# QhelDIV/ShapeFormer

Measured on AMD Instinct MI355X. Metric: shapes/sec completed (64^3 VQDIF + 512-tok AR sample + 128^3 SDF extract), higher is better.
Workload: dtype f32; 1 GPU; shape completion, 384 shapes/GPU/step: VQDIF-16 encode of 16384-pt partial cloud -> tokens -> CondTupleGPT 20+4 layers d1024 prefill + 512 KV-cached decode steps (top_k 100, top_p 0.4, early exit off) -> UNet3D+Upsampler -> 128^3 SDF query; batch_per_gpu=384, micro_batches=4, ar_steps=512, decode_res=128, parallelism=shard1, weights=hash-generated (no checkpoints ship)

## Files before the change

include/sfmi.h:

```cpp
#ifndef SFMI_H
#define SFMI_H
#include <stddef.h>
#ifdef __cplusplus
extern "C" {
#endif

#define SFMI_OK 0
#define SFMI_EINVAL (-1)
#define SFMI_ELDS (-4)
#define SFMI_ENOBLAS (-3)

int sfmi_version(void);
int sfmi_stream_spin(long long ticks, void* stream);
int sfmi_stream_create_cumask(const unsigned* mask, int words, void** stream_out);
int sfmi_stream_destroy(void* stream);
int sfmi_hwid_probe(unsigned* out, int blocks, int threads, long long ticks, void* stream);
int sfmi_tune_set(const char* name, int value);
int sfmi_tune_get(const char* name);
int sfmi_tune_generation(void);

size_t sfmi_enc_pack_floats(void);
int sfmi_enc_pack_weights(const float* fc_pos_w, const float* fc_pos_b, const float* fc0_w, const float* fc0_b,
                          const float* fc1_w, const float* fc1_b, const float* sc_w, const float* fc_c_w,
                          const float* fc_c_b, float* out);
// ... 77 lines not shown
int sfmi_decode_gemm_f32(const float* x, const float* Wp16, const float* c1, const float* c2, const float* resid, float* out,
                         int M, int N, int K, int ldo, int ln, int act, int out_packed, int S, float* slab, int* cnt, void* stream);
int sfmi_decode_gemm_prof_f32(const float* x, const float* Wp16, const float* c1, const float* c2, const float* resid, float* out,
                              int M, int N, int K, int ldo, int ln, int act, int out_packed, int S, float* slab, int* cnt, int* pblk,
                              unsigned long long* prof, void* stream);
int sfmi_decode_gemm_live_f32(const float* x, const float* Wp16, const float* c1, const float* c2, const float* resid, float* out,
                              int M, int N, int K, int ldo, int ln, int act, int out_packed, int S, float* slab, int* cnt,
                              const int* alen, void* stream);
int sfmi_gpt_compact_rows_f32(const int* alen, int* slot_of, int* row_of, int* nlive, int* slot_len, const float* stage, float* resid,
                              int B, int Bpad, int D, void* stream);
int sfmi_decode_gemm_rows_f32(const float* x, const float* Wp16, const float* c1, const float* c2, const float* resid, float* out,
                              int M, int N, int K, int ldo, int ln, int act, int out_packed, int S, float* slab, int* cnt,
                              const int* nlive, int partial, void* stream);
int sfmi_gpt_embed_rows_f32(const float* E0, const float* E1, const float* Ex, const float* pos_emb, const float* cond_pos_emb,
                            const int* seq, const int* len, const int* Lc, float* stage, int B, int D, int Lmax, int end0, void* stream);
int sfmi_gpt_embed_packed_f32(const float* E0, const float* E1, const float* Ex, const float* pos_emb, const float* cond_pos_emb,
                              const int* seq, const int* len, const int* Lc, float* resid, int B, int D, int Lmax, int end0,
                              void* stream);
int sfmi_gpt_attn_decode_f32(const float* qkv_packed, const float* unused, float* Kc, float* Vc, const int* len, float* y_packed,
                             int S, int B, int D, int H, int Lmax, const int* shared_len, void* stream);
int sfmi_gpt_attn_decode_gated_f32(const float* qkv_packed, float* Kc, float* Vc, const int* len, float* y_packed, int B, int D, int H,
                                   int Lmax, const int* shared_len, int* sem, int* blk, int lanes, unsigned long long* prof,
                                   void* stream);
int sfmi_gpt_attn_decode_rows_f32(const float* qkv_packed, float* Kc, float* Vc, const int* slot_len, const int* row_of, float* y_packed,
                                  int B, int D, int H, int Lmax, const int* shared_len, int* sem, int* blk, int lanes,
                                  unsigned long long* prof, void* stream);
int sfmi_gpt_sample_f32(const float* part, int* seq, int* len, const int* Lc, float* logp, float* hist, const int* force,
                        float* resid, const float* E0, const float* E1, const float* Ex, const float* pos_emb, int D, int S,
                        int B, int V, int ldv, int Lmax, int tuple_i, int end0, int end1, int top_k, float top_p,
                        float temperature, int greedy_row0, int mask_invalid, int mask_completion, int max_steps,
// ... 199 lines not shown
```

shapeformer_amd/_lib.py:

```python
from __future__ import annotations

import ctypes as C
import os

_HERE = os.path.dirname(os.path.abspath(__file__))
LIB_PATH = os.path.join(_HERE, "lib", "libsfmi.so")

_lib = None
SFMI_OK, SFMI_EINVAL = 0, -1

c_f32p = C.c_void_p
c_ptr = C.c_void_p
i32, i64, sz, f32 = C.c_int, C.c_longlong, C.c_size_t, C.c_float

PROTOTYPES = {
    "sfmi_version": (i32, []),
    "sfmi_stream_spin": (i32, [i64, c_ptr]),
    "sfmi_stream_create_cumask": (i32, [c_ptr, i32, c_ptr]),
    "sfmi_stream_destroy": (i32, [c_ptr]),
    "sfmi_hwid_probe": (i32, [c_ptr, i32, i32, i64, c_ptr]),
    "sfmi_tune_set": (i32, [C.c_char_p, i32]),
    "sfmi_tune_get": (i32, [C.c_char_p]),
    "sfmi_tune_generation": (i32, []),
    "sfmi_relu_bwd_f32": (i32, [c_ptr, c_ptr, c_ptr, i64, c_ptr]),
# ... 74 lines not shown
                                c_ptr]),
    "sfmi_sgemm_mfma_f32": (i32, [i32] * 5 + [c_ptr, i32, c_ptr, i32, c_ptr, i32, i32, c_ptr, i32, c_ptr, c_ptr, i64, f32, C.c_uint, c_ptr]),
    "sfmi_ce_rows_f32": (i32, [c_ptr, c_ptr, c_ptr, i64, i32, i32, c_ptr]),
    "sfmi_gpt_attn_decode_f32": (i32, [c_ptr] * 6 + [i32] * 5 + [c_ptr, c_ptr]),
    "sfmi_gpt_attn_decode_gated_f32": (i32, [c_ptr] * 5 + [i32] * 4 + [c_ptr, c_ptr, c_ptr, i32, c_ptr, c_ptr]),
    "sfmi_gpt_attn_prefill_f32": (i32, [c_ptr] * 5 + [i32] * 5 + [c_ptr, f32, C.c_uint, c_ptr]),
    "sfmi_gpt_attn_prefill_lse_f32": (i32, [c_ptr] * 5 + [i32] * 5 + [c_ptr, f32, C.c_uint, c_ptr, c_ptr]),
    "sfmi_gpt_sample_f32": (i32, [c_ptr] * 12 + [i32] * 10 + [C.c_float, C.c_float] + [i32] * 4 + [C.c_uint, c_ptr, i32, i32, i32, i32, c_ptr]),
    "sfmi_gpt_sample_live_f32": (i32, [c_ptr] * 12 + [i32] * 10 + [C.c_float, C.c_float] + [i32] * 4 + [C.c_uint, c_ptr, i32, i32, i32, i32, c_ptr, i32,
                                       c_ptr]),
    "sfmi_gpt_mask_logits_f32": (i32, [c_ptr] * 5 + [i32] * 9 + [c_ptr]),
    "sfmi_decode_gemm_f32": (i32, [c_ptr] * 6 + [i32] * 8 + [c_ptr, c_ptr, c_ptr]),
    "sfmi_decode_gemm_live_f32": (i32, [c_ptr] * 6 + [i32] * 8 + [c_ptr, c_ptr, c_ptr, c_ptr]),
    "sfmi_decode_gemm_rows_f32": (i32, [c_ptr] * 6 + [i32] * 8 + [c_ptr, c_ptr, c_ptr, i32, c_ptr]),
    "sfmi_gpt_compact_rows_f32": (i32, [c_ptr] * 7 + [i32] * 3 + [c_ptr]),
    "sfmi_gpt_embed_rows_f32": (i32, [c_ptr] * 9 + [i32] * 4 + [c_ptr]),
    "sfmi_gpt_attn_decode_rows_f32": (i32, [c_ptr] * 6 + [i32] * 4 + [c_ptr, c_ptr, c_ptr, i32, c_ptr, c_ptr]),
    "sfmi_gpt_sample_rows_f32": (i32, [c_ptr] * 11 + [i32] * 10 + [C.c_float, C.c_float] + [i32] * 3 + [C.c_uint, c_ptr, i32, i32, i32, i32, c_ptr, c_ptr,
                                       c_ptr]),
    "sfmi_decode_gemm_prof_f32": (i32, [c_ptr] * 6 + [i32] * 8 + [c_ptr, c_ptr, c_ptr, c_ptr, c_ptr]),
    "sfmi_decode_gemm_slab_floats": (sz, [i32, i32, i32]),
    "sfmi_gpt_embed_packed_f32": (i32, [c_ptr] * 9 + [i32] * 4 + [c_ptr]),
    "sfmi_set_len_i32": (i32, [c_ptr, c_ptr, i32, i32, c_ptr]),
    "sfmi_transpose_f32": (i32, [c_ptr, c_ptr, i32, i32, i32, i32, c_ptr]),
    "sfmi_colsum_f32": (i32, [c_ptr, c_ptr, i32, i32, i32, i32, c_ptr]),
    "sfmi_colsum_slices": (i32, [i32, i32]),
    "sfmi_colsum_ws_f32": (i32, [c_ptr, c_ptr, i32, i32, i32, i32, c_ptr, c_ptr]),
    "sfmi_layernorm_bwd_scratch_floats": (sz, [i32, i32]),
    "sfmi_gelu_f32": (i32, [c_ptr, c_ptr, i64, c_ptr]),
    "sfmi_gelu_bwd_f32": (i32, [c_ptr, c_ptr, c_ptr, i64, c_ptr]),
# ... 110 lines not shown
```

shapeformer_amd/csrc/gpt.hip:

```cpp
#include "sfmi_common.h"
#include <mutex>
#include <type_traits>
#include <string>

#define MFMA(a, b, c) __builtin_amdgcn_mfma_f32_32x32x2f32((a), (b), (c), 0, 0, 0)

#define g_tune g_sfmi_tune


struct RowPrepArgs {
  const float *E0, *E1, *Ex, *pos_emb, *cond_pos_emb;
  const int *seq, *len, *Lc;
  const int* nval;
  const int* extra;
  int* extra_out;
  const float* resid_in;
  const float* part;
  const float* bias;
  const float* Eadd;
  float* resid_out;
  float* xn;
  const float *gamma, *beta;
  int mode, S, M, D, Lmax, P , end0;
  const int* rowoff;
// ... 992 lines not shown
  else {
    int lo = 0, hi = lc;
    while (lo < hi) { int mid = (lo + hi) >> 1; if (row[2 * mid] > pos) hi = mid; else lo = mid + 1; }
    ext = row[2 * (lo < lc ? lo : lc - 1)];
  }
  const f32x4* e0 = reinterpret_cast<const f32x4*>(E0 + (long long)pos * D);
  const f32x4* e1 = reinterpret_cast<const f32x4*>(E1 + (long long)val * D);
  const f32x4* ex = reinterpret_cast<const f32x4*>(Ex + (long long)ext * D);
  const f32x4* pe = reinterpret_cast<const f32x4*>(t < lc ? cond_pos_emb + (long long)t * D : pos_emb + (long long)(t - lc) * D);
  for (int qd = tid; qd < D / 4; qd += 256)
    *reinterpret_cast<f32x4*>(row_major ? resid + (long long)b * D + 4 * qd : resid + pk_off(b, 4 * qd, D)) = ((e0[qd] + e1[qd]) + ex[qd]) + pe[qd];
}

__global__ __launch_bounds__(256) void compact_rows_kernel(const int* __restrict__ alen, int* __restrict__ slot_of, int* __restrict__ row_of,
                                                           int* __restrict__ nlive, int* __restrict__ slot_len,
                                                           const float* __restrict__ stage, float* __restrict__ resid, int B, int Bpad, int D) {
  __shared__ int s_all[4], s_below[4], s_mine;
  const int b = blockIdx.x, tid = threadIdx.x, lane = tid & 63, wave = tid >> 6;
  const int al = tid < B ? alen[tid] : -1;
  const unsigned long long m_all = __ballot(al >= 0), m_below = __ballot(al >= 0 && tid < b);
  if (lane == 0) { s_all[wave] = __popcll(m_all); s_below[wave] = __popcll(m_below); }
  if (tid == b) s_mine = al;
  __syncthreads();
  const int total = (s_all[0] + s_all[1]) + (s_all[2] + s_all[3]), below = (s_below[0] + s_below[1]) + (s_below[2] + s_below[3]);
  const int mine = s_mine;
  const int slot = mine >= 0 ? below : total + (b - below);
  if (tid == 0) {
    slot_of[b] = mine >= 0 ? slot : -1;
    row_of[slot] = b;
    slot_len[slot] = mine >= 0 ? mine : -1;
    if (b == 0) *nlive = total;
  }
  if (b == 0 && B + tid < Bpad) { row_of[B + tid] = -1; slot_len[B + tid] = -1; }
  for (int qd = tid; qd < D / 4; qd += 256) {
    f32x4 v = {0.f, 0.f, 0.f, 0.f};
    if (mine >= 0) v = *reinterpret_cast<const f32x4*>(stage + (long long)b * D + 4 * qd);
    *reinterpret_cast<f32x4*>(resid + pk_off(slot, 4 * qd, D)) = v;
  }
}

__global__ __launch_bounds__(256) void ce_rows_kernel(const float* __restrict__ logits, const int* __restrict__ target,
                                                      float* __restrict__ loss, int V, int ld) {
  __shared__ float red[8];
  const int m = blockIdx.x, tid = threadIdx.x, lane = tid & 63, wave = tid >> 6;
  const float* row = logits + (long long)m * ld;
  float mx = -INFINITY;
// ... 35 lines not shown
  __syncthreads();
  if (part == 0) {
    double a = 0.0, b = 0.0;
    for (int q = 0; q < 16; ++q) { a += p1[r][q]; b += p2[r][q]; }
    if (n < N && bias) b += (double)bias[n];
    c1[nt * 16 + r] = (float)a;
    c2[nt * 16 + r] = (float)b;
  }
}

__global__ void set_len_kernel(int* len, const int* src, int B, int delta) {
  int i = blockIdx.x * blockDim.x + threadIdx.x;
  if (i < B) len[i] = src[i] + delta;
}

template <class P>
static int decode_gemm_launch(const float* x, const float* Wp16, const float* c1, const float* c2, const float* resid, float* out, int M,
                              int N, int K, int ldo, int ln, int act, int out_packed, int S, float* slab, int* cnt, int* pblk,
                              unsigned long long* prof, void* stream, const int* alen = nullptr, const int* nlive = nullptr, int partial = 0) {
  if (prof && (alen || nlive)) return SFMI_EINVAL;
  if (!x || !Wp16 || !out || M <= 0 || M > 192 || S <= 0 || K % S || (ln && !c1)) return SFMI_EINVAL;
  if (out_packed && N % 16) return SFMI_EINVAL;
  if (!out_packed && (ldo < N || ldo % 4)) return SFMI_EINVAL;
  if (S > 1 && (!slab || !cnt)) return SFMI_EINVAL;
  if (prof && !pblk) return SFMI_EINVAL;
  const int kslice = K / S;
  const int tiles = (M + 15) / 16;
  int groups = (tiles + 5) / 6, MT = (tiles + groups - 1) / groups;
  int NWv = (kslice >= 2048 && MT <= 4) ? 16 : 8;
  const int knob_nw = g_tune.dgemm_nw;
  if ((knob_nw == 4 || knob_nw == 8 || knob_nw == 16) && kslice % (16 * knob_nw) == 0 && MT <= (knob_nw == 8 ? 6 : 4)) NWv = knob_nw;
  if (kslice % (16 * NWv)) NWv = kslice % 64 == 0 ? 4 : 1;
  if (kslice % (16 * NWv)) return SFMI_EINVAL;
  const int mt_cap = NWv == 1 ? 1 : NWv == 4 ? 4 : 6;
  if (MT > mt_cap) { groups = (tiles + mt_cap - 1) / mt_cap; MT = (tiles + groups - 1) / groups; }
  DGemmArgs a;
  a.x = x; a.Wp = Wp16; a.c1 = c1; a.c2 = c2; a.resid = resid; a.out = out; a.M = M; a.N = N; a.K = K; a.ldo = ldo; a.ln = ln; a.act = act;
  a.out_packed = out_packed; a.slab = slab; a.cnt = cnt; a.pblk = pblk; a.prof = prof; a.prio = g_tune.dgemm_prio; a.alen = alen;
  a.nlive = nlive; a.partial = partial;
  hipStream_t st = (hipStream_t)stream;
  if ((g_tune.dgemm_nt2 == 2 || (g_tune.dgemm_nt2 == 1 && tiles % 3 == 0)) && NWv == 8 && (kslice / 8 / 16) % 2 == 0 && tiles >= 3) {
    const int g2 = (tiles + 2) / 3, MT2 = (tiles + g2 - 1) / g2;
    dim3 grid2(((N + 15) / 16 + 1) / 2, S, g2);
#define DG2(MT_) hipLaunchKernelGGL((dgemm_kernel<MT_, 8, 2, 2, P>), grid2, dim3(512), 0, st, a)
    if (MT2 == 2) DG2(2); else DG2(3);
#undef DG2
    SFMI_CHECK_LAUNCH();
    return SFMI_OK;
  }
  dim3 grid((N + 15) / 16, S, groups);
  const int steps = kslice / NWv / 16;
  int un = MT == 1 ? 8 : (MT == 2 ? 4 : (MT <= 5 ? 2 : 1));
  if (g_tune.dgemm_un > 0 && g_tune.dgemm_un < un) un = g_tune.dgemm_un;
  while (un & (un - 1)) un &= un - 1;
  while (un > 1 && steps % un) un >>= 1;
#define DG(MT_, NW_, UN_) hipLaunchKernelGGL((dgemm_kernel<MT_, NW_, UN_, 1, P>), grid, dim3(64 * NW_), 0, st, a)
#define DGU8(MT_, NW_) do { if (un >= 8) DG(MT_, NW_, 8); else if (un >= 4) DG(MT_, NW_, 4); else if (un >= 2) DG(MT_, NW_, 2); else DG(MT_, NW_, 1); } while (0)
#define DGU4(MT_, NW_) do { if (un >= 4) DG(MT_, NW_, 4); else if (un >= 2) DG(MT_, NW_, 2); else DG(MT_, NW_, 1); } while (0)
#define DGU2(MT_, NW_) do { if (un >= 2) DG(MT_, NW_, 2); else DG(MT_, NW_, 1); } while (0)
  if (NWv == 16) { if (MT == 1) DGU8(1, 16); else if (MT == 2) DGU4(2, 16); else if (MT == 3) DGU2(3, 16); else DGU2(4, 16); }
  else if (NWv == 4) {
    if (MT == 1) DG(1, 4, 1); else if (MT == 2) DG(2, 4, 1);
    else if (MT == 3) DGU2(3, 4);
    else DGU2(4, 4);
// ... 67 lines not shown
int sfmi_gpt_embed_f32(const float* E0, const float* E1, const float* Ex, const float* pos_emb, const float* cond_pos_emb,
                       const int* seq, const int* len, const int* Lc, const int* nval, const int* extra, int* extra_out,
                       float* resid_out, float* xn, const float* gamma, const float* beta, int B, int P, int D, int Lmax,
                       int end0, const int* rowoff, int M_packed, void* stream) {
  if (!E0 || !E1 || !Ex || !pos_emb || !cond_pos_emb || !seq || !len || !Lc || D % 4 || D > 4096) return SFMI_EINVAL;
  if (rowoff && (P <= 0 || M_packed <= 0)) return SFMI_EINVAL;
  RowPrepArgs a = {};
  a.E0 = E0; a.E1 = E1; a.Ex = Ex; a.pos_emb = pos_emb; a.cond_pos_emb = cond_pos_emb; a.seq = seq; a.len = len; a.Lc = Lc;
  a.nval = nval; a.extra = extra; a.extra_out = extra_out;
  a.resid_out = resid_out; a.xn = xn; a.gamma = gamma; a.beta = beta; a.mode = 0; a.M = P ? B * P : B; a.D = D; a.Lmax = Lmax;
  a.P = P; a.end0 = end0; a.rowoff = rowoff; a.nB = B;
  if (rowoff) a.M = M_packed;
  hipLaunchKernelGGL(rowprep_kernel, dim3(a.M), dim3(256), 0, (hipStream_t)stream, a);
  SFMI_CHECK_LAUNCH();
  return SFMI_OK;
}

int sfmi_gpt_rowprep_f32(const float* resid_in, const float* part, const float* bias, const float* Eadd, const int* seq,
                         const int* len, const int* Lc, const int* nval, float* resid_out, float* xn, const float* gamma,
                         const float* beta, int S, int M, int P, int D, int Lmax, const int* rowoff, int B, void* stream) {
  if (!resid_in || D % 4 || D > 4096 || (Eadd && (!seq || !len)) || (rowoff && B <= 0)) return SFMI_EINVAL;
  RowPrepArgs a = {};
  a.resid_in = resid_in; a.part = part; a.bias = bias; a.Eadd = Eadd; a.seq = seq; a.len = len; a.Lc = Lc; a.nval = nval;
  a.resid_out = resid_out; a.xn = xn; a.gamma = gamma; a.beta = beta; a.mode = 1; a.S = S; a.M = M; a.D = D; a.Lmax = Lmax; a.P = P;
  a.rowoff = rowoff; a.nB = B;
  hipLaunchKernelGGL(rowprep_kernel, dim3(M), dim3(256), 0, (hipStream_t)stream, a);
  SFMI_CHECK_LAUNCH();
  return SFMI_OK;
}

// ... 151 lines not shown
  return SFMI_OK;
}
int sfmi_gpt_embed_rows_f32(const float* E0, const float* E1, const float* Ex, const float* pos_emb, const float* cond_pos_emb,
                            const int* seq, const int* len, const int* Lc, float* stage, int B, int D, int Lmax, int end0, void* stream) {
  if (!E0 || !E1 || !Ex || !pos_emb || !cond_pos_emb || !seq || !len || !Lc || !stage || D % 16) return SFMI_EINVAL;
  hipLaunchKernelGGL(embed_packed_kernel, dim3(B), dim3(256), 0, (hipStream_t)stream, E0, E1, Ex, pos_emb, cond_pos_emb, seq, len, Lc,
                     stage, D, Lmax, end0, 1);
  SFMI_CHECK_LAUNCH();
  return SFMI_OK;
}
int sfmi_gpt_compact_rows_f32(const int* alen, int* slot_of, int* row_of, int* nlive, int* slot_len, const float* stage, float* resid,
                              int B, int Bpad, int D, void* stream) {
  if (!alen || !slot_of || !row_of || !nlive || !slot_len || !stage || !resid || B <= 0 || B > 256 || Bpad < B || Bpad - B > 256 || D % 16)
    return SFMI_EINVAL;
  hipLaunchKernelGGL(compact_rows_kernel, dim3(B), dim3(256), 0, (hipStream_t)stream, alen, slot_of, row_of, nlive, slot_len, stage, resid,
                     B, Bpad, D);
  SFMI_CHECK_LAUNCH();
  return SFMI_OK;
}

int sfmi_ce_rows_f32(const float* logits, const int* target, float* loss, long long M, int V, int ld, void* stream) {
  if (!logits || !target || !loss || M <= 0 || V <= 0) return SFMI_EINVAL;
  hipLaunchKernelGGL(ce_rows_kernel, dim3((unsigned)M), dim3(256), 0, (hipStream_t)stream, logits, target, loss, V, ld);
  SFMI_CHECK_LAUNCH();
  return SFMI_OK;
}

int sfmi_set_len_i32(int* len, const int* src, int B, int delta, void* stream) {
  if (!len || !src) return SFMI_EINVAL;
  hipLaunchKernelGGL(set_len_kernel, dim3((B + 63) / 64), dim3(64), 0, (hipStream_t)stream, len, src, B, delta);
  SFMI_CHECK_LAUNCH();
// ... 5 lines not shown
```

shapeformer_amd/gpt.py:

```python
from __future__ import annotations

import os
import numpy as np
import torch

from . import _lib as L
from . import weights as W


def _t(sd, k, dev):
    v = sd[k]
    if isinstance(v, np.ndarray):
        v = torch.from_numpy(v)
    return v.to(dev, torch.float32).contiguous()


def pack_skinny16(w: torch.Tensor) -> torch.Tensor:
    N, K = w.shape
    NT = (N + 15) // 16
    if NT * 16 != N:
        w = torch.cat([w, w.new_zeros(NT * 16 - N, K)], 0)
    return w.view(NT, 16, K // 16, 4, 4).permute(0, 2, 3, 1, 4).contiguous().view(-1)


class _Layer:
    pass


class CondTupleGPT:
    S_PROJ, S_FC2 = 1, 4
    S_PROJ_M = 1
    PREFILL_ON_CHAIN_STREAMS = True
    PREFILL_BLAS_ROWS = 2048 if os.environ.get("SFMI_ROCBLAS") == "1" else None
    PREFILL_TILE_KERNEL = False

    def _blas(self):
        if not hasattr(self, "_has_blas"):
            self._has_blas = bool(L.lib().sfmi_blas_available())
        return self._has_blas

    def __init__(self, state_dict=None, n_embd=1024, n_head=16, n_layers=(20, 4), block_size=812,
# ... 112 lines not shown

    def mark_decode_weights_stale(self):
        self._decode_stale = True

    def _alloc(self, B, max_steps, slot=0):
        key = (B, max_steps)
        if not hasattr(self, "_states"):
            self._states, self._graphs = {}, {}
        cur = self._states.get(slot)
        if cur is not None and cur["key"] == key:
            self._state = cur
            return cur
        dev, D = self.dev, self.D
        f = lambda *shape: torch.empty(shape, device=dev, dtype=torch.float32)
        Bp = int(L.lib().sfmi_decode_gemm_padded_rows(B))
        st = dict(key=key,
                  seq=torch.zeros(B, self.Lmax + 1, 2, device=dev, dtype=torch.int32),
                  len=torch.zeros(B, device=dev, dtype=torch.int32), Lc=torch.zeros(B, device=dev, dtype=torch.int32),
                  alen=torch.zeros(B, device=dev, dtype=torch.int32),
                  resid=torch.zeros(Bp, D, device=dev), qkv=torch.zeros(Bp, 3 * D, device=dev), y=torch.zeros(Bp, D, device=dev),
                  h=torch.zeros(Bp, 4 * D, device=dev), logit=f(B, self.Vpad),
                  emb=torch.zeros(B, D, device=dev), slot_of=torch.zeros(B, device=dev, dtype=torch.int32),
                  row_of=torch.zeros(Bp, device=dev, dtype=torch.int32), slot_len=torch.zeros(Bp, device=dev, dtype=torch.int32),
                  nlive=torch.zeros(1, device=dev, dtype=torch.int32),
                  slab=f(L.lib().sfmi_decode_gemm_slab_floats(Bp, 4 * D, 4)), cnt=torch.zeros(Bp // 16 * (max(4 * D, self.Vpad) // 16 + 1), device=dev, dtype=torch.int32),
                  Kc=f(len(self.layers), B, self.Lmax + 1, D), Vc=f(len(self.layers), B, self.Lmax + 1, D),
                  logp=torch.zeros(B, max_steps, 2, device=dev, dtype=torch.float32),
                  blk=torch.zeros(1, device=dev, dtype=torch.int32),
                  pblk=torch.zeros(1, device=dev, dtype=torch.int32),
                  prof=self._prof_zero(dev),
                  shared=torch.zeros(1, device=dev, dtype=torch.int32),
                  seed=torch.zeros(1, device=dev, dtype=torch.int32))
        self._state = st
        self._states[slot] = st
        self._graphs.pop(slot, None)
        return st

    @staticmethod
    def _prof_zero(dev):
# ... 3 lines not shown
        return t

    def launch_profile(self, reset=True):
        out = {}
        sts = [st for st in self._states.values() if "prof" in st]
        for i, fam in enumerate(("attn", "gemm")):
            n = sum(int(st["prof"][4 * i + 2].item()) for st in sts)
            tk = sum(int(st["prof"][4 * i + 1].item()) for st in sts)
            out[fam] = (n, tk * 0.01 / n if n else 0.0)
        if reset:
            for st in sts:
                st["prof"].copy_(self._prof_zero(self.dev))
                st["pblk"].zero_()
        return out

    def _dgemm(self, x, wp, c1, c2, resid, out, M, N, K, ldo, ln, act, packed=1, S=1, st=None, prof=False, alen=None, nlive=None, partial=1):
        st = st or self._state
        while S > 1 and (K // S) % 128:
            S //= 2
        slab, cnt = (L.ptr(st["slab"]), L.ptr(st["cnt"])) if S > 1 else (None, None)
        if nlive is not None and not prof:
            L.check(L.lib().sfmi_decode_gemm_rows_f32(L.ptr(x), L.ptr(wp), L.ptr(c1), L.ptr(c2), L.ptr(resid), L.ptr(out), M, N, K, ldo,
                                                      ln, act, packed, S, slab, cnt, L.ptr(nlive), int(partial), L.stream_ptr()), "sfmi_decode_gemm_rows_f32")
            return
        if alen is not None and not prof:
            L.check(L.lib().sfmi_decode_gemm_live_f32(L.ptr(x), L.ptr(wp), L.ptr(c1), L.ptr(c2), L.ptr(resid), L.ptr(out), M, N, K, ldo,
                                                      ln, act, packed, S, slab, cnt, L.ptr(alen), L.stream_ptr()), "sfmi_decode_gemm_live_f32")
            return
        if prof:
            L.check(L.lib().sfmi_decode_gemm_prof_f32(L.ptr(x), L.ptr(wp), L.ptr(c1), L.ptr(c2), L.ptr(resid), L.ptr(out), M, N, K, ldo,
                                                      ln, act, packed, S, slab, cnt, L.ptr(st["pblk"]), L.ptr(st["prof"][4:]),
                                                      L.stream_ptr()), "sfmi_decode_gemm_prof_f32")
            return
        L.check(L.lib().sfmi_decode_gemm_f32(L.ptr(x), L.ptr(wp), L.ptr(c1), L.ptr(c2), L.ptr(resid), L.ptr(out), M, N, K, ldo,
                                             ln, act, packed, S, slab, cnt, L.stream_ptr()), "sfmi_decode_gemm_f32")
# ... 150 lines not shown
            M = lg.shape[0] * lg.shape[1]
            tgt = z[..., i].contiguous().view(-1)
            rows = torch.empty(M, device=self.dev, dtype=torch.float32)
            L.check(L.lib().sfmi_ce_rows_f32(L.ptr(lg), L.ptr(tgt), L.ptr(rows), M, self.V, self.V, L.stream_ptr()), "sfmi_ce_rows_f32")
            loss = loss + rows.mean()
        return loss / 2

    ATTN_LANES = 2
    MAX_CHAIN_ROWS = 192
    SHARED_PREFIX_MIN_ROW_TOKENS = 2800
    SINGLE_CHAIN_ROWS = 96
    SKIP_ENDED = True
    SKIP_ENDED_GEMM = True
    COMPACT_LIVE = True
    COMPACT_LIVE_TILES = True

    def decode_step(self, st, B, sp):
        D = self.D
        lib = L.lib()
        r = st["resid"]
        skip = self._ablate
        if "@" in skip:
            skip = ",".join(t.split("@")[0] for t in skip.split(",") if int(t.split("@")[1]) == sp.get("chain", 0))
        lanes = int(sp.get("gate_lanes", 0))
        pa, pg = "attn" in self._profile, "gemm" in self._profile
        Sqkv, Sproj, Sfc1, Sfc2, Shead = 1, self.S_PROJ if B <= 16 else self.S_PROJ_M, 1, self.S_FC2, 1
        armed = int(sp.get("skip_ended", 0))
        alen_a = st["alen"] if armed else st["len"]
        alen_g = st["alen"] if armed >= 2 else None
        compact = int(sp.get("compact_live", 0))
        gk = dict(alen=alen_g)
        if compact:
            gk = dict(nlive=st["nlive"], partial=int(compact >= 2))
            L.check(lib.sfmi_gpt_compact_rows_f32(L.ptr(st["alen"]), L.ptr(st["slot_of"]), L.ptr(st["row_of"]), L.ptr(st["nlive"]),
                                                  L.ptr(st["slot_len"]), L.ptr(st["emb"]), L.ptr(r), B, r.shape[0], D, L.stream_ptr()),
                    "sfmi_gpt_compact_rows_f32")
        for li, ly in enumerate(self.layers):
            stage_end = li + 1 == len(self.layers) or self.layers[li + 1].stage != ly.stage
            if "gemm" not in skip:
                self._dgemm(r, ly.pqkv, ly.c1qkv, ly.c2qkv, None, st["qkv"], B, 3 * D, D, 3 * D, 1, 0, S=Sqkv, st=st, prof=pg, **gk)
            if "attn" not in skip and compact:
                L.check(lib.sfmi_gpt_attn_decode_rows_f32(L.ptr(st["qkv"]), L.ptr(st["Kc"][li]), L.ptr(st["Vc"][li]),
                                                          L.ptr(st["slot_len"]), L.ptr(st["row_of"]), L.ptr(st["y"]), B, D, self.H, self.Lmax + 1,
                                                          L.ptr(st["shared"]) if sp.get("shared_prefix") else None,
                                                          L.ptr(self._sem) if lanes else None, L.ptr(st["blk"]) if (lanes or pa) else None, lanes,
                                                          L.ptr(st["prof"]) if pa else None, L.stream_ptr()), "sfmi_gpt_attn_decode_rows_f32")
            elif "attn" not in skip:
                L.check(lib.sfmi_gpt_attn_decode_gated_f32(L.ptr(st["qkv"]), L.ptr(st["Kc"][li]), L.ptr(st["Vc"][li]),
                                                           L.ptr(alen_a), L.ptr(st["y"]), B, D, self.H, self.Lmax + 1,
                                                           L.ptr(st["shared"]) if sp.get("shared_prefix") else None,
                                                           L.ptr(self._sem) if lanes else None, L.ptr(st["blk"]) if (lanes or pa) else None, lanes,
                                                           L.ptr(st["prof"]) if pa else None, L.stream_ptr()), "sfmi_gpt_attn_decode_gated_f32")
            if "gemm" not in skip:
                self._dgemm(st["y"], ly.pproj, None, ly.bproj, r, r, B, D, D, D, 0, 0, S=Sproj, st=st, prof=pg, **gk)
                self._dgemm(r, ly.pfc1, ly.c1fc1, ly.c2fc1, None, st["h"], B, 4 * D, D, 4 * D, 1, 1, S=Sfc1, st=st, prof=pg, **gk)
                self._dgemm(st["h"], ly.pfc2, None, ly.bfc2, r, r, B, D, 4 * D, D, 0, 0, S=Sfc2, st=st, prof=pg, **gk)
            if stage_end:
                s = ly.stage
# ... 24 lines not shown
    def _prepare(self, c_tokens, Lc, max_steps, sp_kw, slot=0, row_offset=0, rows_total=None, return_logits=False,
                 force_tokens=None, use_graph=True, shared_prefix=False, z_tokens=None, gate_lanes=0):
        B = c_tokens.shape[0]
        Lz = 0 if z_tokens is None else int(z_tokens.shape[1])
        if B > self.MAX_CHAIN_ROWS:
            raise L.SfmiError(f"a decode chain holds up to {self.MAX_CHAIN_ROWS} rows (larger batches run as several chains: sample / sample_microbatched)")
        self._sync_params()
        if getattr(self, "_decode_stale", False):
            self.refresh_decode_weights()
        Lc_host = Lc.cpu().tolist()
        Lc_max = max(Lc_host)
        if shared_prefix == "auto":
            shared_prefix = B * Lc_max >= self.SHARED_PREFIX_MIN_ROW_TOKENS
        steps = min(max_steps, self.Lmax - Lc_max - Lz)
        st = self._alloc(B, max_steps, slot)
        st["seq"].zero_()
        st["seq"][:, :c_tokens.shape[1]] = c_tokens.to(self.dev, torch.int32)
        st["Lc"].copy_(Lc.to(self.dev, torch.int32))
        st["len"].copy_(st["Lc"])
        if Lz:
            pos = st["Lc"].long()[:, None] + torch.arange(Lz, device=self.dev)[None, :]
            st["seq"][torch.arange(B, device=self.dev)[:, None], pos] = torch.as_tensor(z_tokens).to(self.dev, torch.int32)
            st["len"].add_(Lz)
            shared_prefix = False
        st["alen"].copy_(st["len"])
        st["slot_of"].copy_(torch.arange(B, device=self.dev, dtype=torch.int32))
        st["row_of"].fill_(-1)
        st["row_of"][:B] = st["slot_of"]
        st["slot_len"].fill_(-1)
        st["slot_len"][:B] = st["len"]
        st["nlive"].fill_(B)
        st["logp"].zero_()
        st["seed"].copy_(torch.from_numpy(np.array([sp_kw["seed"]], np.uint32).view(np.int32)))
        hist = None
        if return_logits:
            hist = [torch.full((B, max_steps, self.V), float("nan"), device=self.dev) for _ in range(2)]
        sp = dict(sp_kw, max_steps=int(max_steps), hist=hist, row_offset=int(row_offset),
                  rows_total=int(rows_total if rows_total is not None else B), chain=int(slot - 100 if slot >= 100 else 0),
                  shared_prefix=bool(shared_prefix), step_offset=Lz, gate_lanes=int(gate_lanes))
        sp["skip_ended"] = (2 if self.SKIP_ENDED_GEMM else 1) if (self.SKIP_ENDED and sp_kw["mask_invalid"] and not return_logits
                                                                  and force_tokens is None and not self._ablate) else 0
        sp["compact_live"] = (2 if self.COMPACT_LIVE_TILES else 1) if (self.COMPACT_LIVE and sp["skip_ended"] >= 2) else 0
        if force_tokens is not None:
            ft = torch.zeros(B, max_steps, 2, dtype=torch.int32)
            ft[:, :force_tokens.shape[1]] = torch.as_tensor(force_tokens).to(torch.int32)
            sp["force"] = ft.to(self.dev)
            use_graph = False
        P = Lc_max + Lz - 1
        st["nval"], st["extra"] = None, None
        if Lz:
            st["nval"] = (st["len"] - 1).contiguous()
        if shared_prefix:
            assert len(set(Lc_host)) == 1 and bool((st["seq"][:, :Lc_max] == st["seq"][:1, :Lc_max]).all()), \
                "shared_prefix needs identical condition rows"
            st["shared"].fill_(P)
            st["M_packed"] = P
            st["rowoff"] = torch.tensor([0, P], dtype=torch.int32).to(self.dev)
# ... 4 lines not shown
            nrow = [max(l + Lz - 1, 0) for l in Lc_host]
            st["M_packed"] = sum(nrow)
            st["rowoff"] = torch.tensor([0] + list(np.cumsum(nrow)), dtype=torch.int32).to(self.dev)
            if P > 0 and st["M_packed"] > 0:
                self.prefill(st, B, P)
        if sp["compact_live"]:
            L.check(L.lib().sfmi_gpt_embed_rows_f32(L.ptr(self.E[0]), L.ptr(self.E[1]), L.ptr(self.Ex), L.ptr(self.pos_emb),
                                                    L.ptr(self.cond_pos_emb), L.ptr(st["seq"]), L.ptr(st["len"]), L.ptr(st["Lc"]),
                                                    L.ptr(st["emb"]), B, self.D, self.Lmax + 1, self.end[0], L.stream_ptr()),
                    "sfmi_gpt_embed_rows_f32")
        else:
            L.check(L.lib().sfmi_gpt_embed_packed_f32(L.ptr(self.E[0]), L.ptr(self.E[1]), L.ptr(self.Ex), L.ptr(self.pos_emb),
                                                      L.ptr(self.cond_pos_emb), L.ptr(st["seq"]), L.ptr(st["len"]), L.ptr(st["Lc"]),
                                                      L.ptr(st["resid"]), B, self.D, self.Lmax + 1, self.end[0], L.stream_ptr()),
                    "sfmi_gpt_embed_packed_f32")
        graph = None
        if use_graph and steps > 1:
            gkey = (B, tuple(sorted((k, v) for k, v in sp.items() if k not in ("hist", "force", "seed"))), return_logits,
                    self._ablate, self._profile, self.S_PROJ, self.S_PROJ_M, self.S_FC2,
                    int(L.lib().sfmi_tune_generation()))
            cached = self._graphs.get(slot)
            if cached is None or cached[0] != gkey or return_logits:
                side = torch.cuda.Stream(device=self.dev)
                side.wait_stream(torch.cuda.current_stream())
                saved = {k: st[k].clone() for k in ("seq", "len", "alen", "logp", "resid", "emb")}
                with torch.cuda.stream(side):
                    self.decode_step(st, B, sp)
                torch.cuda.current_stream().wait_stream(side)
                torch.cuda.synchronize()
                for k, v in saved.items():
                    st[k].copy_(v)
                graph = torch.cuda.CUDAGraph()
                with torch.cuda.graph(graph):
                    self.decode_step(st, B, sp)
                for k, v in saved.items():
                    st[k].copy_(v)
                self._graphs[slot] = (gkey, graph)
            graph = self._graphs[slot][1]
        return dict(st=st, sp=sp, B=B, steps=steps, graph=graph, hist=hist, Lc_host=Lc_host, Lz=Lz)

    @staticmethod
    def _sp(top_k, top_p, temperature, best_in_first, mask_invalid, mask_invalid_completion, seed):
        return dict(top_k=int(top_k), top_p=float(top_p), temperature=float(temperature), best_in_first=best_in_first,
                    mask_invalid=mask_invalid, mask_invalid_completion=mask_invalid_completion,
                    seed=W._fnv1a32(f"sample-uniforms-{seed}"))

    @torch.no_grad()
    def sample(self, c_tokens, Lc, max_steps=512, top_k=100, top_p=0.4, temperature=1.0, best_in_first=True,
               mask_invalid=True, mask_invalid_completion=True, seed=0, stop_early=True, use_graph=True,
               return_logits=False, check_every=32, force_tokens=None, to_host=True, after_prefill=None, shared_prefix=False,
               z_tokens=None, row_offset=0, rows_total=None, ended_reduce=None):
        if c_tokens.shape[0] > self.SINGLE_CHAIN_ROWS:
            n_micro = min(4, -(-c_tokens.shape[0] // 80))
            r = self.sample_microbatched(c_tokens, Lc, n_micro=n_micro, max_steps=max_steps, top_k=top_k, top_p=top_p, temperature=temperature,
# ... 4 lines not shown
                                         ended_reduce=ended_reduce)
            if not to_host:
                return r
            Lz = 0 if z_tokens is None else int(z_tokens.shape[1])
            return self._host_result(r["state"], Lc.cpu().tolist(), Lz, r.get("logits_history"))
        sp_kw = self._sp(top_k, top_p, temperature, best_in_first, mask_invalid, mask_invalid_completion, seed)
        ctx = self._prepare(c_tokens, Lc, max_steps, sp_kw, return_logits=return_logits, force_tokens=force_tokens,
                            use_graph=use_graph, shared_prefix=shared_prefix, z_tokens=z_tokens, row_offset=int(row_offset),
                            rows_total=rows_total)
        ended = (lambda: self._all_ended(st, B)) if ended_reduce is None else (lambda: bool(ended_reduce(self._all_ended(st, B))))
        st, sp, B, steps, g, hist, Lc_host = (ctx[k] for k in ("st", "sp", "B", "steps", "graph", "hist", "Lc_host"))
        if after_prefill is not None:
            after_prefill()
        done = 0
        if g is not None:
            while done < steps:
                n = min(check_every, steps - done) if stop_early else steps - done
                for _ in range(n):
                    g.replay()
                done += n
                if stop_early and ended():
                    break
        else:
            while done < steps:
                self.decode_step(st, B, sp)
                done += 1
                if stop_early and (done % check_every == 0 or done == steps) and ended():
                    break
        if not to_host:
            return dict(state=st, steps=done)
        return self._host_result(st, Lc_host, ctx["Lz"], hist)

    def _host_result(self, st, Lc_host, Lz, hist):
        B = len(Lc_host)
        ln = st["len"].cpu().tolist()
# ... 124 lines not shown
        if lanes:
            for s in streams:
                cur.wait_stream(s)
            self._sem.zero_()
            for c in ctxs:
                c["st"]["blk"].zero_()
            for s in streams:
                s.wait_stream(cur)
        if after_prefill is not None:
            for s in streams:
                cur.wait_stream(s)
            after_prefill()
            for s in streams:
                s.wait_stream(cur)
        done = 0
        while done < steps:
            n = min(check_every, steps - done) if stop_early else steps - done
            for _ in range(n):
                for c, s in zip(ctxs, streams):
                    with torch.cuda.stream(s):
                        if c["graph"] is not None:
                            c["graph"].replay()
                        else:
                            self.decode_step(c["st"], c["B"], c["sp"])
            done += n
            if stop_early:
                for s in streams:
                    cur.wait_stream(s)
                e_ = all(self._all_ended(c["st"], c["B"]) for c in ctxs)
                if (e_ if ended_reduce is None else bool(ended_reduce(e_))):
                    break
        for s in streams:
            cur.wait_stream(s)
        merged = {k: torch.cat([c["st"][k] for c in ctxs], 0) for k in ("seq", "len", "Lc", "logp")}
        res = dict(state=merged, steps=done)
        if return_logits:
            res["logits_history"] = [torch.cat([c["hist"][i] for c in ctxs], 0) for i in range(2)]
        return res

    def _all_ended(self, st, B):
# ... 5 lines not shown
```

Before: 139.6 shapes/s.

## Capture per-tile-budget decode graphs and pick one from lagged live-row feedback

Captures one decode-step graph for each row-tile budget and selects the budget every 8 steps. The choice uses the live-row count read back asynchronously from two intervals earlier through a pinned ring and events. Decode GEMMs and attention then launch only the budgeted row tiles, so grid size shrinks as sequences end, instead of relying on in-kernel skipping. It adds graph capture time and memory plus periodic host event syncs. An overflow flag raises an error if live rows ever exceed the budget, which could happen if the lag assumption breaks.

```diff
diff --git a/include/sfmi.h b/include/sfmi.h
--- a/include/sfmi.h
+++ b/include/sfmi.h
@@ -115,6 +115,11 @@
                               const int* nlive, int partial, void* stream);
 int sfmi_gpt_embed_rows_f32(const float* E0, const float* E1, const float* Ex, const float* pos_emb, const float* cond_pos_emb,
                             const int* seq, const int* len, const int* Lc, float* stage, int B, int D, int Lmax, int end0, void* stream);
+int sfmi_decode_gemm_tiles_f32(const float* x, const float* Wp16, const float* c1, const float* c2, const float* resid, float* out,
+                               int form_rows, int tiles, int N, int K, int ldo, int ln, int act, int out_packed, int S, float* slab,
+                               int* cnt, const int* nlive, int partial, void* stream);
+int sfmi_gpt_compact_rows_budget_f32(const int* alen, int* slot_of, int* row_of, int* nlive, int* slot_len, const float* stage,
+                                     float* resid, int B, int Bpad, int D, int budget, int* over, void* stream);
 int sfmi_gpt_embed_packed_f32(const float* E0, const float* E1, const float* Ex, const float* pos_emb, const float* cond_pos_emb,
                               const int* seq, const int* len, const int* Lc, float* resid, int B, int D, int Lmax, int end0,
                               void* stream);
diff --git a/shapeformer_amd/_lib.py b/shapeformer_amd/_lib.py
--- a/shapeformer_amd/_lib.py
+++ b/shapeformer_amd/_lib.py
@@ -112,6 +112,8 @@
     "sfmi_decode_gemm_live_f32": (i32, [c_ptr] * 6 + [i32] * 8 + [c_ptr, c_ptr, c_ptr, c_ptr]),
     "sfmi_decode_gemm_rows_f32": (i32, [c_ptr] * 6 + [i32] * 8 + [c_ptr, c_ptr, c_ptr, i32, c_ptr]),
     "sfmi_gpt_compact_rows_f32": (i32, [c_ptr] * 7 + [i32] * 3 + [c_ptr]),
+    "sfmi_decode_gemm_tiles_f32": (i32, [c_ptr] * 6 + [i32] * 9 + [c_ptr, c_ptr, c_ptr, i32, c_ptr]),
+    "sfmi_gpt_compact_rows_budget_f32": (i32, [c_ptr] * 7 + [i32] * 4 + [c_ptr, c_ptr]),
     "sfmi_gpt_embed_rows_f32": (i32, [c_ptr] * 9 + [i32] * 4 + [c_ptr]),
     "sfmi_gpt_attn_decode_rows_f32": (i32, [c_ptr] * 6 + [i32] * 4 + [c_ptr, c_ptr, c_ptr, i32, c_ptr, c_ptr]),
     "sfmi_gpt_sample_rows_f32": (i32, [c_ptr] * 11 + [i32] * 10 + [C.c_float, C.c_float] + [i32] * 3 + [C.c_uint, c_ptr, i32, i32, i32, i32, c_ptr, c_ptr,
diff --git a/shapeformer_amd/csrc/gpt.hip b/shapeformer_amd/csrc/gpt.hip
--- a/shapeformer_amd/csrc/gpt.hip
+++ b/shapeformer_amd/csrc/gpt.hip
@@ -1030,7 +1030,8 @@
 
 __global__ __launch_bounds__(256) void compact_rows_kernel(const int* __restrict__ alen, int* __restrict__ slot_of, int* __restrict__ row_of,
                                                            int* __restrict__ nlive, int* __restrict__ slot_len,
-                                                           const float* __restrict__ stage, float* __restrict__ resid, int B, int Bpad, int D) {
+                                                           const float* __restrict__ stage, float* __restrict__ resid, int B, int Bpad, int D,
+                                                           int budget, int* __restrict__ over) {
   __shared__ int s_all[4], s_below[4], s_mine;
   const int b = blockIdx.x, tid = threadIdx.x, lane = tid & 63, wave = tid >> 6;
   const int al = tid < B ? alen[tid] : -1;
@@ -1045,7 +1046,10 @@
     slot_of[b] = mine >= 0 ? slot : -1;
     row_of[slot] = b;
     slot_len[slot] = mine >= 0 ? mine : -1;
-    if (b == 0) *nlive = total;
+    if (b == 0) {
+      *nlive = total;
+      if (over && total > 16 * budget) over[0] = 1;
+    }
   }
   if (b == 0 && B + tid < Bpad) { row_of[B + tid] = -1; slot_len[B + tid] = -1; }
   for (int qd = tid; qd < D / 4; qd += 256) {
@@ -1111,10 +1115,12 @@
   if (i < B) len[i] = src[i] + delta;
 }
 
+extern "C" int sfmi_decode_gemm_padded_rows(int M);
 template <class P>
 static int decode_gemm_launch(const float* x, const float* Wp16, const float* c1, const float* c2, const float* resid, float* out, int M,
                               int N, int K, int ldo, int ln, int act, int out_packed, int S, float* slab, int* cnt, int* pblk,
-                              unsigned long long* prof, void* stream, const int* alen = nullptr, const int* nlive = nullptr, int partial = 0) {
+                              unsigned long long* prof, void* stream, const int* alen = nullptr, const int* nlive = nullptr, int partial = 0,
+                              int budget = 0) {
   if (prof && (alen || nlive)) return SFMI_EINVAL;
   if (!x || !Wp16 || !out || M <= 0 || M > 192 || S <= 0 || K % S || (ln && !c1)) return SFMI_EINVAL;
   if (out_packed && N % 16) return SFMI_EINVAL;
@@ -1122,22 +1128,27 @@
   if (S > 1 && (!slab || !cnt)) return SFMI_EINVAL;
   if (prof && !pblk) return SFMI_EINVAL;
   const int kslice = K / S;
-  const int tiles = (M + 15) / 16;
+  int tiles = (M + 15) / 16;
   int groups = (tiles + 5) / 6, MT = (tiles + groups - 1) / groups;
   int NWv = (kslice >= 2048 && MT <= 4) ? 16 : 8;
   const int knob_nw = g_tune.dgemm_nw;
   if ((knob_nw == 4 || knob_nw == 8 || knob_nw == 16) && kslice % (16 * knob_nw) == 0 && MT <= (knob_nw == 8 ? 6 : 4)) NWv = knob_nw;
   if (kslice % (16 * NWv)) NWv = kslice % 64 == 0 ? 4 : 1;
   if (kslice % (16 * NWv)) return SFMI_EINVAL;
-  const int mt_cap = NWv == 1 ? 1 : NWv == 4 ? 4 : 6;
+  if (budget > 0) {
+    tiles = budget;
+    groups = (tiles + 5) / 6; MT = (tiles + groups - 1) / groups;
+  }
+  const int mt_cap = NWv == 1 ? 1 : (NWv == 4 || NWv == 16) ? 4 : 6;
   if (MT > mt_cap) { groups = (tiles + mt_cap - 1) / mt_cap; MT = (tiles + groups - 1) / groups; }
   DGemmArgs a;
-  a.x = x; a.Wp = Wp16; a.c1 = c1; a.c2 = c2; a.resid = resid; a.out = out; a.M = M; a.N = N; a.K = K; a.ldo = ldo; a.ln = ln; a.act = act;
+  a.x = x; a.Wp = Wp16; a.c1 = c1; a.c2 = c2; a.resid = resid; a.out = out; a.M = budget > 0 ? min(M, 16 * budget) : M; a.N = N; a.K = K; a.ldo = ldo; a.ln = ln; a.act = act;
   a.out_packed = out_packed; a.slab = slab; a.cnt = cnt; a.pblk = pblk; a.prof = prof; a.prio = g_tune.dgemm_prio; a.alen = alen;
   a.nlive = nlive; a.partial = partial;
   hipStream_t st = (hipStream_t)stream;
   if ((g_tune.dgemm_nt2 == 2 || (g_tune.dgemm_nt2 == 1 && tiles % 3 == 0)) && NWv == 8 && (kslice / 8 / 16) % 2 == 0 && tiles >= 3) {
     const int g2 = (tiles + 2) / 3, MT2 = (tiles + g2 - 1) / g2;
+    if (budget > 0 && g2 * MT2 * 16 > sfmi_decode_gemm_padded_rows(M)) return SFMI_EINVAL;
     dim3 grid2(((N + 15) / 16 + 1) / 2, S, g2);
 #define DG2(MT_) hipLaunchKernelGGL((dgemm_kernel<MT_, 8, 2, 2, P>), grid2, dim3(512), 0, st, a)
     if (MT2 == 2) DG2(2); else DG2(3);
@@ -1145,6 +1156,7 @@
     SFMI_CHECK_LAUNCH();
     return SFMI_OK;
   }
+  if (budget > 0 && groups * MT * 16 > sfmi_decode_gemm_padded_rows(M)) return SFMI_EINVAL;
   dim3 grid((N + 15) / 16, S, groups);
   const int steps = kslice / NWv / 16;
   int un = MT == 1 ? 8 : (MT == 2 ? 4 : (MT <= 5 ? 2 : 1));
@@ -1242,6 +1254,14 @@
   hipLaunchKernelGGL(rowprep_kernel, dim3(a.M), dim3(256), 0, (hipStream_t)stream, a);
   SFMI_CHECK_LAUNCH();
   return SFMI_OK;
+}
+
+int sfmi_decode_gemm_tiles_f32(const float* x, const float* Wp16, const float* c1, const float* c2, const float* resid,
+                               float* out, int form_rows, int tiles, int N, int K, int ldo, int ln, int act, int out_packed, int S,
+                               float* slab, int* cnt, const int* nlive, int partial, void* stream) {
+  if (!nlive || form_rows <= 0 || form_rows > 192 || tiles < 1 || 16 * tiles > sfmi_decode_gemm_padded_rows(form_rows)) return SFMI_EINVAL;
+  return decode_gemm_launch<DgProduct>(x, Wp16, c1, c2, resid, out, form_rows, N, K, ldo, ln, act, out_packed, S, slab, cnt, nullptr, nullptr,
+                                       stream, nullptr, nlive, partial ? 1 : 0, tiles);
 }
 
 int sfmi_gpt_rowprep_f32(const float* resid_in, const float* part, const float* bias, const float* Eadd, const int* seq,
@@ -1423,7 +1443,17 @@
   if (!alen || !slot_of || !row_of || !nlive || !slot_len || !stage || !resid || B <= 0 || B > 256 || Bpad < B || Bpad - B > 256 || D % 16)
     return SFMI_EINVAL;
   hipLaunchKernelGGL(compact_rows_kernel, dim3(B), dim3(256), 0, (hipStream_t)stream, alen, slot_of, row_of, nlive, slot_len, stage, resid,
-                     B, Bpad, D);
+                     B, Bpad, D, 0, (int*)nullptr);
+  SFMI_CHECK_LAUNCH();
+  return SFMI_OK;
+}
+int sfmi_gpt_compact_rows_budget_f32(const int* alen, int* slot_of, int* row_of, int* nlive, int* slot_len, const float* stage, float* resid,
+                                     int B, int Bpad, int D, int budget, int* over, void* stream) {
+  if (!alen || !slot_of || !row_of || !nlive || !slot_len || !stage || !resid || B <= 0 || B > 256 || Bpad < B || Bpad - B > 256 || D % 16)
+    return SFMI_EINVAL;
+  if (!over || budget < 1 || 16 * budget > Bpad) return SFMI_EINVAL;
+  hipLaunchKernelGGL(compact_rows_kernel, dim3(B), dim3(256), 0, (hipStream_t)stream, alen, slot_of, row_of, nlive, slot_len, stage, resid,
+                     B, Bpad, D, budget, over);
   SFMI_CHECK_LAUNCH();
   return SFMI_OK;
 }
diff --git a/shapeformer_amd/gpt.py b/shapeformer_amd/gpt.py
--- a/shapeformer_amd/gpt.py
+++ b/shapeformer_amd/gpt.py
@@ -25,6 +25,55 @@
 
 class _Layer:
     pass
+
+
+def tile_budget_policy(full, nlive_of_block, block, lag=2):
+    if block < lag:
+        return int(full)
+    return int(min(int(full), max(1, (int(nlive_of_block[block - lag]) + 15) // 16)))
+
+
+class _BudgetFeedback:
+    RING = 4
+
+    def __init__(self, gpt, ctxs, streams):
+        self.ctxs, self.streams, self.every = ctxs, streams, max(1, int(gpt.TILE_BUDGET_EVERY))
+        self.armed = [c.get("graphs") is not None for c in ctxs]
+        self.cur = [c["graph"] for c in ctxs]
+        self.seen = [[] for _ in ctxs]
+        if any(self.armed):
+            self.ring = [torch.zeros(self.RING, 2, dtype=torch.int32).pin_memory() if a else None for a in self.armed]
+            self.ev = [[torch.cuda.Event() for _ in range(self.RING)] if a else None for a in self.armed]
+        for c in ctxs:
+            c["budget_log"] = []
+        gpt.last_budget_log = [c["budget_log"] for c in ctxs]
+
+    def graphs(self, done):
+        if done % self.every == 0:
+            j = done // self.every
+            for i, c in enumerate(self.ctxs):
+                if not self.armed[i]:
+                    continue
+                if j >= 2:
+                    self.ev[i][(j - 2) % self.RING].synchronize()
+                    nlive, over = self.ring[i][(j - 2) % self.RING].tolist()
+                    if over:
+                        raise L.SfmiError("a decode step ran at a row-tile budget below its live rows (TILE_BUDGET)")
+                    self.seen[i].append(nlive)
+                T = tile_budget_policy((c["B"] + 15) // 16, self.seen[i], j)
+                c["budget_log"].append(T)
+                self.cur[i] = c["graphs"][T]
+        return self.cur
+
+    def stepped(self, done):
+        if (done + 1) % self.every:
+            return
+        k = (done // self.every) % self.RING
+        for i, (c, s) in enumerate(zip(self.ctxs, self.streams)):
+            if self.armed[i]:
+                with torch.cuda.stream(s):
+                    self.ring[i][k].copy_(c["st"]["nlo"], non_blocking=True)
+                    self.ev[i][k].record(s)
 
 
 class CondTupleGPT:
@@ -167,6 +216,7 @@
         dev, D = self.dev, self.D
         f = lambda *shape: torch.empty(shape, device=dev, dtype=torch.float32)
         Bp = int(L.lib().sfmi_decode_gemm_padded_rows(B))
+        nlo = torch.zeros(2, device=dev, dtype=torch.int32)
         st = dict(key=key,
                   seq=torch.zeros(B, self.Lmax + 1, 2, device=dev, dtype=torch.int32),
                   len=torch.zeros(B, device=dev, dtype=torch.int32), Lc=torch.zeros(B, device=dev, dtype=torch.int32),
@@ -175,7 +225,7 @@
                   h=torch.zeros(Bp, 4 * D, device=dev), logit=f(B, self.Vpad),
                   emb=torch.zeros(B, D, device=dev), slot_of=torch.zeros(B, device=dev, dtype=torch.int32),
                   row_of=torch.zeros(Bp, device=dev, dtype=torch.int32), slot_len=torch.zeros(Bp, device=dev, dtype=torch.int32),
-                  nlive=torch.zeros(1, device=dev, dtype=torch.int32),
+                  nlo=nlo, nlive=nlo[:1], over=nlo[1:],
                   slab=f(L.lib().sfmi_decode_gemm_slab_floats(Bp, 4 * D, 4)), cnt=torch.zeros(Bp // 16 * (max(4 * D, self.Vpad) // 16 + 1), device=dev, dtype=torch.int32),
                   Kc=f(len(self.layers), B, self.Lmax + 1, D), Vc=f(len(self.layers), B, self.Lmax + 1, D),
                   logp=torch.zeros(B, max_steps, 2, device=dev, dtype=torch.float32),
@@ -209,11 +259,15 @@
                 st["pblk"].zero_()
         return out
 
-    def _dgemm(self, x, wp, c1, c2, resid, out, M, N, K, ldo, ln, act, packed=1, S=1, st=None, prof=False, alen=None, nlive=None, partial=1):
+    def _dgemm(self, x, wp, c1, c2, resid, out, M, N, K, ldo, ln, act, packed=1, S=1, st=None, prof=False, alen=None, nlive=None, partial=1, tiles=0):
         st = st or self._state
         while S > 1 and (K // S) % 128:
             S //= 2
         slab, cnt = (L.ptr(st["slab"]), L.ptr(st["cnt"])) if S > 1 else (None, None)
+        if nlive is not None and not prof and tiles:
+            L.check(L.lib().sfmi_decode_gemm_tiles_f32(L.ptr(x), L.ptr(wp), L.ptr(c1), L.ptr(c2), L.ptr(resid), L.ptr(out), M, int(tiles), N, K, ldo,
+                                                       ln, act, packed, S, slab, cnt, L.ptr(nlive), int(partial), L.stream_ptr()), "sfmi_decode_gemm_tiles_f32")
+            return
         if nlive is not None and not prof:
             L.check(L.lib().sfmi_decode_gemm_rows_f32(L.ptr(x), L.ptr(wp), L.ptr(c1), L.ptr(c2), L.ptr(resid), L.ptr(out), M, N, K, ldo,
                                                       ln, act, packed, S, slab, cnt, L.ptr(nlive), int(partial), L.stream_ptr()), "sfmi_decode_gemm_rows_f32")
@@ -394,8 +448,11 @@
     SKIP_ENDED_GEMM = True
     COMPACT_LIVE = True
     COMPACT_LIVE_TILES = True
-
-    def decode_step(self, st, B, sp):
+    TILE_BUDGET = True
+    TILE_BUDGET_EVERY = 8
+    TILE_BUDGET_FORMS = None
+
+    def decode_step(self, st, B, sp, budget=0):
         D = self.D
         lib = L.lib()
         r = st["resid"]
@@ -410,7 +467,16 @@
         alen_g = st["alen"] if armed >= 2 else None
         compact = int(sp.get("compact_live", 0))
         gk = dict(alen=alen_g)
-        if compact:
+        Ba = B
+        if compact >= 2 and budget:
+            gk = dict(nlive=st["nlive"], partial=1, tiles=int(budget))
+            Ba = min(B, 16 * int(budget))
+            L.check(lib.sfmi_gpt_compact_rows_budget_f32(L.ptr(st["alen"]), L.ptr(st["slot_of"]), L.ptr(st["row_of"]), L.ptr(st["nlive"]),
+                                                         L.ptr(st["slot_len"]), L.ptr(st["emb"]), L.ptr(r), B, r.shape[0], D, int(budget),
+                                                         L.ptr(st["over"]), L.stream_ptr()), "sfmi_gpt_compact_rows_budget_f32")
+        elif budget:
+            raise L.SfmiError("a row-tile budget needs a packed chain that runs live row tiles only")
+        elif compact:
             gk = dict(nlive=st["nlive"], partial=int(compact >= 2))
             L.check(lib.sfmi_gpt_compact_rows_f32(L.ptr(st["alen"]), L.ptr(st["slot_of"]), L.ptr(st["row_of"]), L.ptr(st["nlive"]),
                                                   L.ptr(st["slot_len"]), L.ptr(st["emb"]), L.ptr(r), B, r.shape[0], D, L.stream_ptr()),
@@ -421,7 +487,7 @@
                 self._dgemm(r, ly.pqkv, ly.c1qkv, ly.c2qkv, None, st["qkv"], B, 3 * D, D, 3 * D, 1, 0, S=Sqkv, st=st, prof=pg, **gk)
             if "attn" not in skip and compact:
                 L.check(lib.sfmi_gpt_attn_decode_rows_f32(L.ptr(st["qkv"]), L.ptr(st["Kc"][li]), L.ptr(st["Vc"][li]),
-                                                          L.ptr(st["slot_len"]), L.ptr(st["row_of"]), L.ptr(st["y"]), B, D, self.H, self.Lmax + 1,
+                                                          L.ptr(st["slot_len"]), L.ptr(st["row_of"]), L.ptr(st["y"]), Ba, D, self.H, self.Lmax + 1,
                                                           L.ptr(st["shared"]) if sp.get("shared_prefix") else None,
                                                           L.ptr(self._sem) if lanes else None, L.ptr(st["blk"]) if (lanes or pa) else None, lanes,
                                                           L.ptr(st["prof"]) if pa else None, L.stream_ptr()), "sfmi_gpt_attn_decode_rows_f32")
@@ -476,6 +542,9 @@
             shared_prefix = B * Lc_max >= self.SHARED_PREFIX_MIN_ROW_TOKENS
         steps = min(max_steps, self.Lmax - Lc_max - Lz)
         st = self._alloc(B, max_steps, slot)
+        if self.TILE_BUDGET and int(st["over"].item()):
+            st["over"].zero_()
+            raise L.SfmiError("a decode step ran at a row-tile budget below its live rows (TILE_BUDGET): the last results of this chain are invalid")
         st["seq"].zero_()
         st["seq"][:, :c_tokens.shape[1]] = c_tokens.to(self.dev, torch.int32)
         st["Lc"].copy_(Lc.to(self.dev, torch.int32))
@@ -503,6 +572,7 @@
         sp["skip_ended"] = (2 if self.SKIP_ENDED_GEMM else 1) if (self.SKIP_ENDED and sp_kw["mask_invalid"] and not return_logits
                                                                   and force_tokens is None and not self._ablate) else 0
         sp["compact_live"] = (2 if self.COMPACT_LIVE_TILES else 1) if (self.COMPACT_LIVE and sp["skip_ended"] >= 2) else 0
+        sp["tile_budget"] = int(bool(self.TILE_BUDGET and sp["compact_live"] == 2 and "gemm" not in self._profile))
         if force_tokens is not None:
             ft = torch.zeros(B, max_steps, 2, dtype=torch.int32)
             ft[:, :force_tokens.shape[1]] = torch.as_tensor(force_tokens).to(torch.int32)
@@ -537,30 +607,41 @@
                                                       L.ptr(self.cond_pos_emb), L.ptr(st["seq"]), L.ptr(st["len"]), L.ptr(st["Lc"]),
                                                       L.ptr(st["resid"]), B, self.D, self.Lmax + 1, self.end[0], L.stream_ptr()),
                     "sfmi_gpt_embed_packed_f32")
-        graph = None
+        graph, graphs = None, None
         if use_graph and steps > 1:
+            full = (B + 15) // 16
+            forms = tuple(sorted(set(self.TILE_BUDGET_FORMS))) if self.TILE_BUDGET_FORMS is not None else None
             gkey = (B, tuple(sorted((k, v) for k, v in sp.items() if k not in ("hist", "force", "seed"))), return_logits,
-                    self._ablate, self._profile, self.S_PROJ, self.S_PROJ_M, self.S_FC2,
+                    self._ablate, self._profile, self.S_PROJ, self.S_PROJ_M, self.S_FC2, forms,
                     int(L.lib().sfmi_tune_generation()))
             cached = self._graphs.get(slot)
             if cached is None or cached[0] != gkey or return_logits:
                 side = torch.cuda.Stream(device=self.dev)
-                side.wait_stream(torch.cuda.current_stream())
-                saved = {k: st[k].clone() for k in ("seq", "len", "alen", "logp", "resid", "emb")}
-                with torch.cuda.stream(side):
-                    self.decode_step(st, B, sp)
-                torch.cuda.current_stream().wait_stream(side)
-                torch.cuda.synchronize()
-                for k, v in saved.items():
-                    st[k].copy_(v)
-                graph = torch.cuda.CUDAGraph()
-                with torch.cuda.graph(graph):
-                    self.decode_step(st, B, sp)
-                for k, v in saved.items():
-                    st[k].copy_(v)
-                self._graphs[slot] = (gkey, graph)
+                saved = {k: st[k].clone() for k in ("seq", "len", "alen", "logp", "resid", "emb", "over")}
+
+                def capture(budget):
+                    side.wait_stream(torch.cuda.current_stream())
+                    with torch.cuda.stream(side):
+                        self.decode_step(st, B, sp, budget)
+                    torch.cuda.current_stream().wait_stream(side)
+                    torch.cuda.synchronize()
+                    for k, v in saved.items():
+                        st[k].copy_(v)
+                    g_ = torch.cuda.CUDAGraph()
+                    with torch.cuda.graph(g_):
+                        self.decode_step(st, B, sp, budget)
+                    for k, v in saved.items():
+                        st[k].copy_(v)
+                    return g_
+                graph = capture(0)
+                by_budget = {full: graph}
+                if sp["tile_budget"]:
+                    for T in range(full - 1, 0, -1):
+                        by_budget[T] = capture(T) if (forms is None or T in forms) else by_budget[T + 1]
+                self._graphs[slot] = (gkey, graph, by_budget)
             graph = self._graphs[slot][1]
-        return dict(st=st, sp=sp, B=B, steps=steps, graph=graph, hist=hist, Lc_host=Lc_host, Lz=Lz)
+            graphs = self._graphs[slot][2] if sp["tile_budget"] else None
+        return dict(st=st, sp=sp, B=B, steps=steps, graph=graph, graphs=graphs, budget_log=[], hist=hist, Lc_host=Lc_host, Lz=Lz)
 
     @staticmethod
     def _sp(top_k, top_p, temperature, best_in_first, mask_invalid, mask_invalid_completion, seed):
@@ -595,11 +676,13 @@
             after_prefill()
         done = 0
         if g is not None:
+            fb = _BudgetFeedback(self, [ctx], [torch.cuda.current_stream()])
             while done < steps:
                 n = min(check_every, steps - done) if stop_early else steps - done
                 for _ in range(n):
-                    g.replay()
-                done += n
+                    fb.graphs(done)[0].replay()
+                    fb.stepped(done)
+                    done += 1
                 if stop_early and ended():
                     break
         else:
@@ -754,16 +837,22 @@
             for s in streams:
                 s.wait_stream(cur)
         done = 0
+        fb = _BudgetFeedback(self, ctxs, streams)
+        on_step = getattr(self, "_on_step", None)
         while done < steps:
             n = min(check_every, steps - done) if stop_early else steps - done
             for _ in range(n):
-                for c, s in zip(ctxs, streams):
+                gs = fb.graphs(done)
+                for c, s, g_ in zip(ctxs, streams, gs):
                     with torch.cuda.stream(s):
-                        if c["graph"] is not None:
-                            c["graph"].replay()
+                        if g_ is not None:
+                            g_.replay()
                         else:
                             self.decode_step(c["st"], c["B"], c["sp"])
-            done += n
+                fb.stepped(done)
+                done += 1
+                if on_step is not None:
+                    on_step(done, streams)
             if stop_early:
                 for s in streams:
                     cur.wait_stream(s)
```

Result: faster. 152.8 shapes/s (median of 6 runs) (+9.5%).
